# tokkiwa/FlashGMM

Measured on AMD Instinct MI355X. Metric: encode+decode Mpixels/s (Kodak, K=4 N=192) + GMM-CDF HBM GB/s vs roofline, higher is better.
Workload: dtype f32; 1 GPU; kodak24; schedule=codec, images_per_gpu=24, K=4, approx_mode=polya, param_dtype=f32, coded_symbols_per_gpu=6223104, streams_per_gpu=48, one_device_rehearsal=False

## Files before the change

flashgmm_amd/csrc/fgmm_capi.cpp:

```cpp
#include <sched.h>

#include <string>

#include "fgmm_ctx.h"

using namespace fgmm;

namespace fgmm {

static thread_local char t_err[512] = "";
char *last_error_buffer(size_t *cap) {
  if (cap) *cap = sizeof t_err;
  return t_err;
}
int fail(int code, const char *fmt, ...) {
  va_list ap;
  va_start(ap, fmt);
  vsnprintf(t_err, sizeof t_err, fmt, ap);
  va_end(ap);
  return code;
}

}

// ... 87 lines not shown
  m.ms[5] = tr.ms();
  m.worker_busy_ms = busy;
  m.worker_wait_ms = wait;
  for (int k = 0; k < 3; ++k) m.head_ms[k] = head ? head[k] : 0.0;
}
int fgmm_ctx::prof_begin(int which, dev::Stream s) {
  if (!profiling) return FGMM_OK;
  DEV_TRY(dev::event_record(prof[which][0], s));
  return FGMM_OK;
}
int fgmm_ctx::prof_end(int which, dev::Stream s) {
  if (!profiling) return FGMM_OK;
  DEV_TRY(dev::event_record(prof[which][1], s));
  prof_valid[which] = true;
  return FGMM_OK;
}

namespace {
bool mode_ok(int mode) { return mode >= 0 && mode <= 2; }
struct StagedRows {
  const float *s = nullptr, *m = nullptr, *w = nullptr;
  int64_t stride_n = 0, stride_k = 0;
};
}

extern "C" {

int fgmm_abi_version(void) { return FGMM_ABI_VERSION; }
const char *fgmm_last_error(void) { return fgmm::last_error_buffer(nullptr); }

namespace {
struct OptName {
  const char *name;
  int64_t fgmm_ctx::Opts::*field;
  int64_t lo, hi;
  const char *env;
};
const OptName kOpts[] = {
    {"pieces", &fgmm_ctx::Opts::pieces, 0, kMaxPieces, "FGMM_PIECES"},
    {"dec_first", &fgmm_ctx::Opts::dec_first, 1, 1 << 20, "FGMM_DEC_FIRST"},
    {"tab_cap_e", &fgmm_ctx::Opts::tab_cap_e, 256, 32768, "FGMM_TAB_CAP_E"},
    {"stage_max_mb", &fgmm_ctx::Opts::stage_max_mb, 0, 1 << 30, "FGMM_STAGE_MAX_MB"},
    {"trace", &fgmm_ctx::Opts::trace, 0, 2, "FGMM_TRACE"},
    {"enc_vec", &fgmm_ctx::Opts::enc_vec, 0, 8, "FGMM_VEC"},
    {"enc_linear", &fgmm_ctx::Opts::enc_linear, 0, 1, nullptr},
    {"ef_rows", &fgmm_ctx::Opts::ef_rows, 0, 2, "FGMM_EF_ROWS"},
    {"ef_min", &fgmm_ctx::Opts::ef_min, kTabEfMin, 1 << 20, "FGMM_EF_MIN_ROWS"},
    {"enc_ways", &fgmm_ctx::Opts::enc_ways, 0, kMaxEncWays, "FGMM_ENC_WAYS"},
    {"ckpt_decode", &fgmm_ctx::Opts::ckpt_decode, 0, 2, "FGMM_CKPT_DECODE"},
    {"spin_lat", &fgmm_ctx::Opts::spin_lat, -1, 1ll << 40, "FGMM_SPIN_LAT"},
    {"gpu_decode", &fgmm_ctx::Opts::gpu_decode, 0, 2, "FGMM_GPU_DECODE"},
    {"enc_segs", &fgmm_ctx::Opts::enc_segs, 0, 2, "FGMM_ENC_SEGS"},
    {"scatter_rounds", &fgmm_ctx::Opts::scatter_rounds, 0, 1, nullptr},
};
}

namespace {
double cgroup_cpu_quota() {
  double best = -1.0;
  auto take = [&best](double q) {
    if (q > 0 && (best < 0 || q < best)) best = q;
  };
  auto read_line = [](const std::string &path, char *buf, size_t cap) {
    FILE *f = fopen(path.c_str(), "r");
    if (!f) return false;
    const bool ok = fgets(buf, (int)cap, f) != nullptr;
    fclose(f);
    return ok;
  };
  char buf[256];
  std::string v2_rel, v1_rel;
  const std::string sysroot = getenv("FGMM_SYSROOT") ? getenv("FGMM_SYSROOT") : "";
  if (FILE *f = fopen((sysroot + "/proc/self/cgroup").c_str(), "r")) {
    while (fgets(buf, sizeof buf, f)) {
      std::string ln(buf);
      while (!ln.empty() && (ln.back() == '\n' || ln.back() == '\r')) ln.pop_back();
      const size_t a = ln.find(':'), b = a == std::string::npos ? a : ln.find(':', a + 1);
      if (b == std::string::npos) continue;
      const std::string ctrl = ln.substr(a + 1, b - a - 1), rel = ln.substr(b + 1);
      if (ctrl.empty()) v2_rel = rel;
      else if (("," + ctrl + ",").find(",cpu,") != std::string::npos) v1_rel = rel;
    }
    fclose(f);
  }
  for (const char *root : {"/sys/fs/cgroup", "/sys/fs/cgroup/unified"}) {
    std::string rel = v2_rel;
    for (;;) {
      if (read_line(sysroot + root + rel + (rel.empty() || rel.back() != '/' ? "/" : "") + "cpu.max", buf, sizeof buf)) {
        long long q = 0, p = 0;
        if (sscanf(buf, "%lld %lld", &q, &p) == 2 && q > 0 && p > 0) take((double)q / (double)p);
      }
      if (rel.empty() || rel == "/") break;
      const size_t cut = rel.find_last_of('/');
      rel = cut == std::string::npos ? std::string() : rel.substr(0, cut);
    }
  }
  for (const char *root : {"/sys/fs/cgroup/cpu", "/sys/fs/cgroup/cpu,cpuacct"}) {
    std::string rel = v1_rel;
    for (;;) {
      const std::string dir = sysroot + root + rel + (rel.empty() || rel.back() != '/' ? "/" : "");
      long long q = 0, p = 0;
      if (read_line(dir + "cpu.cfs_quota_us", buf, sizeof buf) && sscanf(buf, "%lld", &q) == 1 && q > 0 &&
          read_line(dir + "cpu.cfs_period_us", buf, sizeof buf) && sscanf(buf, "%lld", &p) == 1 && p > 0)
        take((double)q / (double)p);
      if (rel.empty() || rel == "/") break;
      const size_t cut = rel.find_last_of('/');
// ... 835 lines not shown
```

flashgmm_amd/csrc/fgmm_ctx.h:

```cpp
#pragma once
#include <math.h>
#include <pthread.h>
#include <sched.h>
#include <stdarg.h>
#include <stdio.h>
#include <stdlib.h>
#include <string.h>

#include <algorithm>
#include <atomic>
#include <chrono>
#include <condition_variable>
#include <functional>
#include <mutex>
#include <queue>
#include <string>
#include <thread>
#include <vector>

#include "../../include/flashgmm_amd.h"
#include "fgmm_device.h"
#include "fgmm_internal.h"

namespace fgmm {
// ... 240 lines not shown
CensusOff census_take(Arena &ar, int M);
void census_bind(EncDesc &d, const fgmm_ctx *ctx, const CensusOff &o);
void census_desc(EncDesc &d, const fgmm_ctx *ctx, const CensusOff &o, const float *y, const fgmm_params *params_or_null, int M, int64_t hw,
                 int clamp);
bool enc_vec4_ok(const EncDesc &d, const void *out, bool two_byte);
int census_side_info(const fgmm_ctx *ctx, const CensusOff &o, int M, int64_t hw, int64_t *zero_bitmap_or_null, int32_t *abs_max_out,
                     float *min_max_or_null = nullptr);

struct DeviceGuard {
  int prev = -1;
  bool ok = false;
  explicit DeviceGuard(int d) {
    if (dev::get_device(&prev) == 0 && (prev == d || dev::set_device(d) == 0)) ok = true;
  }
  ~DeviceGuard() {
    int cur;
    if (ok && prev >= 0 && dev::get_device(&cur) == 0 && cur != prev) (void)dev::set_device(prev);
  }
};

struct TempDevice {
  std::vector<void *> v;
  ~TempDevice() {
    for (void *p : v) (void)dev::free_device(p);
  }
  int alloc(size_t bytes, char **out) {
    void *p = nullptr;
    DEV_TRY(dev::malloc_device(&p, std::max<size_t>(bytes, 256)));
    v.push_back(p);
    *out = static_cast<char *>(p);
    return FGMM_OK;
  }
};

}

struct fgmm_ctx {
  int device = 0;
  std::mutex mu;
  fgmm::Pool *pool = nullptr;
  fgmm::WorkerCpus worker_cpus;
  fgmm::Pool *dec_pool = nullptr;
  fgmm::Pool *decoders() const { return dec_pool ? dec_pool : pool; }
  char *d_ws = nullptr;
  size_t d_cap = 0;
  char *h_ws = nullptr;
  size_t h_cap = 0;
  std::vector<fgmm::dev::Event> events;
  std::vector<fgmm::dev::Event> sleep_events;
  fgmm::dev::Stream copy_stream = nullptr;
  fgmm::dev::Stream aux_stream = nullptr;
  struct Opts {
    int64_t pieces = 0, dec_first = 2, tab_cap_e = fgmm::kTabCapE, stage_max_mb = 0, trace = 0, enc_vec = 0, enc_linear = 1, ef_rows = 0,
            ef_min = fgmm::kTabEfDefault, enc_ways = 0, ckpt_decode = 0, spin_lat = 400000, gpu_decode = 0, enc_segs = 1, scatter_rounds = 1;
  } opt;
  struct Chunk {
    char *p;
    size_t cap, used;
  };
  std::vector<Chunk> chunks;
  void chunks_reset() {
    for (auto &c : chunks) c.used = 0;
  }
  int chunk_alloc(size_t bytes, char **out);
  char *d_stage = nullptr;
  size_t d_stage_cap = 0;
  int ensure_stage(size_t bytes);
  void *d_xs = nullptr;
  size_t d_xs_cap = 0;
  uint32_t *d_rate_log2 = nullptr;
  size_t stage_budget() const;
  int ensure_streams();
  int ensure_device(size_t bytes);
  int ensure_host(size_t bytes);
  int ensure_events(size_t n, size_t n_sleep = 0);
  std::vector<int32_t> h_sym;
  void trim();
  const std::chrono::steady_clock::time_point born = std::chrono::steady_clock::now();
  static constexpr int kLogCap = 64;
  fgmm_call_marks log[kLogCap];
  unsigned long long log_n = 0;
  void log_call(int kind, int count, const fgmm::Trace &tr, const double ms[5], double busy, double wait, const double *head = nullptr);
  bool profiling = false;
  fgmm::dev::Event prof[4][2] = {{nullptr, nullptr}, {nullptr, nullptr}, {nullptr, nullptr}, {nullptr, nullptr}};
  bool prof_valid[4] = {false, false, false, false};
  int prof_begin(int which, fgmm::dev::Stream s);
  int prof_end(int which, fgmm::dev::Stream s);
  unsigned long long stat[6] = {0, 0, 0, 0, 0, 0};
};

namespace fgmm {

struct EncItem {
  bool latent = false;
  const float *y = nullptr;
  const float *x = nullptr;
  const void *xs = nullptr;
  const int32_t *sym_dev = nullptr;
  const int32_t *sym_host = nullptr;
  fgmm_params prm{};
  int64_t stride_p = 1;
  int32_t M = 0;
  int64_t hw = 0;
  int clamp = 0;
  float *yq = nullptr;
  fgmm_symbuf *symbuf = nullptr;
  int64_t ckpt_stride = 0;
// ... 164 lines not shown
```

flashgmm_amd/csrc/fgmm_decode_gpu.cpp:

```cpp
#include "fgmm_ctx.h"

namespace fgmm {

bool gpu_decodable(const DecItem &it, int64_t n) {
  return it.y_hat && !it.sym_host_out && it.ckpt && it.n_ckpt > 0 && it.ckpt_stride >= 256 && !(it.ckpt_stride & (it.ckpt_stride - 1)) &&
         n > 0 && it.n_ckpt == (n - 1) / it.ckpt_stride && it.n_ckpt < (1 << 24) && it.max_bs >= 0 && 2 * (int64_t)it.max_bs + 2 <= 2048  &&
         it.enc_len >= 8 && !(it.enc_len & 3) && it.stride_p == 1;
}

int decode_batch_gpu(fgmm_ctx *ctx, dev::Stream stream, std::vector<DecItem> &items, const std::vector<int> &which, int mode,
                     std::vector<int> &redo) {
  Trace tr("decode-gpu", (int)ctx->opt.trace);
  const int count = (int)which.size();
  const bool clamped = items[which[0]].clamp != 0, f16 = items[which[0]].prm.dtype == FGMM_F16;
  Arena ar;
  int64_t n_segs = 0;
  for (int k = 0; k < count; ++k) n_segs += items[which[k]].n_ckpt + 1;
  const size_t o_descs = ar.take(sizeof(SegDesc) * (size_t)count);
  const size_t o_segs = ar.take(sizeof(SegRef) * (size_t)n_segs);
  struct Off {
    size_t list, ckpt, words, status;
  };
  std::vector<Off> off((size_t)count);
  for (int k = 0; k < count; ++k) {
    DecItem &it = items[which[k]];
    off[(size_t)k].list = ar.take(sizeof(int32_t) * (size_t)std::max(it.M, 1), 16);
    off[(size_t)k].ckpt = ar.take(sizeof(fgmm_ckpt) * (size_t)it.n_ckpt, 16);
    off[(size_t)k].words = ar.take(it.enc_len, 16);
  }
  const size_t upload_bytes = ar.off;
  const size_t o_status = ar.take(sizeof(uint32_t) * (size_t)n_segs, 256);
  {
    size_t at = o_status;
    for (int k = 0; k < count; ++k) {
      off[(size_t)k].status = at;
      at += sizeof(uint32_t) * (size_t)(items[which[k]].n_ckpt + 1);
    }
  }
  int rc;
  if ((rc = ctx->ensure_device(ar.off)) || (rc = ctx->ensure_host(ar.off))) return rc;
  SegDesc *hd = reinterpret_cast<SegDesc *>(ctx->h_ws + o_descs);
  SegRef *hs = reinterpret_cast<SegRef *>(ctx->h_ws + o_segs);
  int64_t max_dead = 0;
  for (int k = 0; k < count; ++k) {
    DecItem &it = items[which[k]];
    int32_t *list = reinterpret_cast<int32_t *>(ctx->h_ws + off[(size_t)k].list);
    int r = 0, dead = it.n_ch;
    for (int c = 0; c < it.M; ++c) {
      if (!it.zero_bitmap || it.zero_bitmap[c] != 0) list[r++] = c;
      else list[dead++] = c;
    }
    max_dead = std::max<int64_t>(max_dead, it.M - it.n_ch);
    memcpy(ctx->h_ws + off[(size_t)k].ckpt, it.ckpt, sizeof(fgmm_ckpt) * (size_t)it.n_ckpt);
    memcpy(ctx->h_ws + off[(size_t)k].words, it.enc, it.enc_len);
    SegDesc &d = hd[k];
    memset(&d, 0, sizeof d);
    d.scales = it.prm.scales;
    d.means = it.prm.means;
    d.weights = it.prm.weights;
    d.stride_k = it.prm.stride_k;
    d.stride_c = it.prm.stride_c;
    d.stride_p = it.stride_p;
    d.hw = it.hw;
    d.n = it.n;
    d.chan_list = reinterpret_cast<const int32_t *>(ctx->d_ws + off[(size_t)k].list);
    d.max_bs = it.max_bs;
    d.clamp = it.clamp;
    d.logits = (it.prm.flags & FGMM_PARAMS_LOGITS) ? 1 : 0;
    d.words = reinterpret_cast<const uint32_t *>(ctx->d_ws + off[(size_t)k].words);
    d.n_words = (int64_t)(it.enc_len / 4);
    d.ckpt = reinterpret_cast<const fgmm_ckpt *>(ctx->d_ws + off[(size_t)k].ckpt);
    d.n_ckpt = it.n_ckpt;
    d.stride = it.ckpt_stride;
    d.y_hat = it.y_hat;
    d.status = reinterpret_cast<uint32_t *>(ctx->d_ws + off[(size_t)k].status);
    d.dead_list = d.chan_list + it.n_ch;
    d.n_dead = it.M - it.n_ch;
  }
  {
    constexpr int kBuckets = 256;
    std::vector<uint32_t> wgt((size_t)n_segs);
    uint32_t w_max = 1;
    int64_t at = 0;
    for (int k = 0; k < count; ++k) {
      const DecItem &it = items[which[k]];
      const uint64_t end_all = it.enc_len / 4 - 2;
      uint64_t prev = 0;
      for (int64_t sgm = 0; sgm <= it.n_ckpt; ++sgm) {
        const uint64_t pos = sgm < it.n_ckpt ? it.ckpt[sgm].pos : end_all;
        const uint64_t wds = pos >= prev ? pos - prev : 0;
        wgt[(size_t)at] = (uint32_t)std::min<uint64_t>(wds, 0x7FFFFFFFu);
        w_max = std::max(w_max, wgt[(size_t)at]);
        prev = pos;
        ++at;
      }
    }
    int64_t first[kBuckets + 1] = {};
    auto bucket = [&](uint32_t wv) { return kBuckets - 1 - (int)((uint64_t)wv * (kBuckets - 1) / w_max); };
    for (int64_t q = 0; q < n_segs; ++q) ++first[bucket(wgt[(size_t)q]) + 1];
    for (int b = 0; b < kBuckets; ++b) first[b + 1] += first[b];
    at = 0;
    for (int k = 0; k < count; ++k)
      for (int64_t sgm = 0; sgm <= items[which[k]].n_ckpt; ++sgm, ++at) hs[first[bucket(wgt[(size_t)at])]++] = SegRef{k, (int32_t)sgm};
  }
  DEV_TRY(dev::copy_async(ctx->d_ws, ctx->h_ws, upload_bytes, dev::kH2D, stream));
  LAUNCH_TRY(launch_segzero(reinterpret_cast<const SegDesc *>(ctx->d_ws + o_descs), count, max_dead, stream));
  if ((rc = ctx->prof_begin(3, stream))) return rc;
  LAUNCH_TRY(launch_segdec(reinterpret_cast<const SegDesc *>(ctx->d_ws + o_descs), reinterpret_cast<const SegRef *>(ctx->d_ws + o_segs), n_segs, mode_with_planes(mode, items[which[0]].prm.dtype),
                           clamped, f16, stream));
  if ((rc = ctx->prof_end(3, stream))) return rc;
  DEV_TRY(dev::copy_async(ctx->h_ws + o_status, ctx->d_ws + o_status, sizeof(uint32_t) * (size_t)n_segs, dev::kD2H, stream));
  tr.mark("enqueued");
  const double t_enq = tr.ms();
  DEV_TRY(dev::stream_sync(stream));
  tr.mark("segments decoded");
  {
    const double t_done = tr.ms(), mk[5] = {t_enq, t_enq, t_enq, t_done, t_done};
    ctx->log_call(2, count, tr, mk, 0.0, 0.0);
  }
  for (int k = 0; k < count; ++k) {
    DecItem &it = items[which[k]];
    const uint32_t *st = reinterpret_cast<const uint32_t *>(ctx->h_ws + off[(size_t)k].status);
    uint32_t worst = 0;
    for (int64_t sgm = 0; sgm <= it.n_ckpt; ++sgm) worst = std::max(worst, st[sgm]);
    if (worst != kSegOk) redo.push_back(which[k]);
    else it.status = FGMM_OK, it.done.store(1);
    if (tr.on && worst != kSegOk) {
      int64_t first = 0, n_bad = 0;
      for (int64_t sgm = it.n_ckpt; sgm >= 0; --sgm)
        if (st[sgm] != kSegOk) first = sgm, ++n_bad;
      fprintf(stderr, "[fgmm decode-gpu]   item %d: %lld of %lld segments not ok, the first: segment %lld status %u\n", which[k], (long long)n_bad,
              (long long)it.n_ckpt + 1, (long long)first, st[first]);
    }
  }
  ctx->stat[1] = 0;
  ctx->stat[2] = ctx->stat[3] = 0;
  ctx->stat[4] = (unsigned long long)(count - (int)redo.size());
  ctx->stat[5] = (unsigned long long)redo.size();
  for (int k = 0; k < count; ++k) ctx->stat[2] += (unsigned long long)items[which[k]].n;
  return FGMM_OK;
}

}
```

flashgmm_amd/csrc/fgmm_internal.h:

```cpp
#pragma once
#include <stddef.h>
#include <stdint.h>

#include "../../include/flashgmm_amd.h"

#if defined(__HIPCC__)
#define FGMM_HD __host__ __device__
#else
#define FGMM_HD
#endif

namespace fgmm {


struct EncDesc {
  const float *y;
  const int32_t *sym;
  const void *scales, *means, *weights;
  int64_t stride_k, stride_c, stride_p;
  int64_t hw;
  int32_t M;
  int32_t clamp;
  int32_t logits;
  uint32_t meta_slots;
// ... 93 lines not shown
  const float *anchors;
  float *out;
  const float *wp, *bp;
  int32_t M, c_out, h, w2, odd;
  int32_t mt, n_kt;
  int32_t pt;
};
int launch_ckbd_ctx_pack(const float *w, const float *bias_or_null, int M, int c_out, bool transposed, float *wp, float *bp, uint32_t *bad, void *stream);
int ckbd_ctx_tiles(int64_t n, int64_t pt, int c_out);
int launch_ckbd_ctx(const CkbdCtxArgs &args, int64_t n, void *stream);

constexpr int kCkbdWgradSliceMin = 256;
constexpr int kCkbdWgradSliceMax = 16;
struct CkbdWgradSlices { int64_t S, L; };
static inline CkbdWgradSlices ckbd_wgrad_slices(int64_t P) {
  if (P <= 0) return {0, 32};
  const int64_t want = (P + kCkbdWgradSliceMin - 1) / kCkbdWgradSliceMin, s0 = want < kCkbdWgradSliceMax ? want : kCkbdWgradSliceMax;
  const int64_t L = 32 * ((P + 32 * s0 - 1) / (32 * s0));
  return {(P + L - 1) / L, L};
}
static inline int64_t ckbd_wgrad_cols(int M) { return (int64_t)kCkbdCtxTaps * M + 1; }
struct CkbdWgradArgs {
  const float *anchors, *g;
  float *partial;
  int32_t M, c_out, h, w2, odd;
  int32_t mt;
  int32_t col0, n_col;
  int32_t P, L, S;
};
int ckbd_wgrad_tiles(int64_t S, int n_col, int c_out);
int launch_ckbd_wgrad(const CkbdWgradArgs &args, void *stream);
int launch_ckbd_wgrad_finish(const float *partial, int M, int c_out, int S, float *dweight_or_null, float *dbias_or_null, void *stream);

struct SegDesc {
  const void *scales, *means, *weights;
  int64_t stride_k, stride_c, stride_p;
  int64_t hw;
  int64_t n;
  const int32_t *chan_list;
  int32_t max_bs, clamp, logits, pad_;
  const uint32_t *words;
  int64_t n_words;
  const fgmm_ckpt *ckpt;
  int64_t n_ckpt, stride;
  float *y_hat;
  uint32_t *status;
  const int32_t *dead_list;
  int64_t n_dead;
};
struct SegRef {
  int32_t item, seg;
};
enum : uint32_t { kSegOk = 0, kSegMismatch = 1, kSegHard = 2, kSegStream = 3 };
int launch_segdec(const SegDesc *d_descs, const SegRef *d_segs, int64_t n_segs, int mode, bool clamped, bool f16, void *stream);
int launch_segzero(const SegDesc *d_descs, int count, int64_t max_dead, void *stream);

constexpr int kMaxPieces = 32;
constexpr int kAutoPiecesMax = 24;
constexpr int kEncSegs = 4;
constexpr int kTabEdgeSlots = 64;
constexpr int kTabCounters = 4 + kTabEdgeSlots;
#ifndef FGMM_EF_MIN
#define FGMM_EF_MIN 14
#endif
constexpr uint32_t kTabEfMin = FGMM_EF_MIN;
constexpr uint32_t kTabEfDefault = 33;
constexpr uint32_t kHdr2Escape = 255;
FGMM_HD static inline int32_t cvtt_i32(float f) {
  return (f > -2147483904.0f && f < 2147483648.0f) ? (int32_t)f : INT32_MIN;
}
FGMM_HD static inline uint32_t tab_hdr_pack(int32_t a, uint32_t cnt, uint32_t nonmono) {
  return (uint32_t)(uint16_t)(int16_t)a | ((cnt & 0x7FFFu) << 16) | (nonmono << 31);
}
FGMM_HD static inline int32_t tab_hdr_a(uint32_t h) { return (int32_t)(int16_t)(uint16_t)(h & 0xFFFFu); }
FGMM_HD static inline uint32_t tab_hdr_cnt(uint32_t h) { return (h >> 16) & 0x7FFFu; }
FGMM_HD static inline uint32_t tab_hdr_nonmono(uint32_t h) { return h >> 31; }
FGMM_HD static inline unsigned long long tab_hdr8_pack(int32_t a, uint32_t cnt, uint32_t nonmono) {
  return (unsigned long long)(uint32_t)a | ((unsigned long long)((cnt & 0x7FFFFFFFu) | (nonmono << 31)) << 32);
}
FGMM_HD static inline int32_t tab_hdr8_a(unsigned long long h) { return (int32_t)(uint32_t)h; }
FGMM_HD static inline uint32_t tab_hdr8_cnt(unsigned long long h) { return (uint32_t)(h >> 32) & 0x7FFFFFFFu; }
FGMM_HD static inline uint32_t tab_hdr8_nonmono(unsigned long long h) { return (uint32_t)(h >> 63); }
constexpr uint32_t kTabNoEf = 0x7FFFFFFFu;
FGMM_HD static inline bool tab_row_is_ef(uint32_t cnt, uint32_t nonmono, uint32_t ef_min) { return cnt >= ef_min && !nonmono; }
constexpr uint32_t kTabEf12Max = 48;
FGMM_HD static inline uint32_t tab_ef_l(uint32_t cnt) { return cnt <= kTabEf12Max ? 12u : 8u; }
FGMM_HD static inline uint32_t tab_ef_hb(uint32_t cnt, uint32_t l) { return cnt + (65536u >> l); }
FGMM_HD static inline uint32_t tab_ef_lb(uint32_t cnt, uint32_t l) { return (tab_ef_hb(cnt, l) + 7u) & ~7u; }
FGMM_HD static inline unsigned long long tab_ef_bits(uint32_t cnt, uint32_t l) { return (unsigned long long)cnt * l + tab_ef_lb(cnt, l); }
FGMM_HD static inline unsigned long long tab_row_bytes(uint32_t cnt, uint32_t nonmono, uint32_t ef_min) {
  return tab_row_is_ef(cnt, nonmono, ef_min) ? 2ull * ((tab_ef_bits(cnt, tab_ef_l(cnt)) + 15ull) >> 4) : 2ull * (unsigned long long)cnt;
}
FGMM_HD static inline bool tab_hdr_fits16(int32_t max_bs) { return 2 * (int64_t)max_bs + 2 <= 254; }
FGMM_HD static inline int tab_hdr_form(int32_t max_bs) { return tab_hdr_fits16(max_bs) ? 2 : (max_bs <= 16382 ? 4 : 8); }
constexpr int kTabCapE = 12288;
constexpr int kTabCapEWide = 16384;
constexpr int kTabMaxTl = 256;
FGMM_HD static inline int tab_tl(int32_t max_bs, int cap_e) {
  const int64_t W = 2 * (int64_t)max_bs + 2;
  const int64_t t = (cap_e / W) & ~15ll;
  return t >= 16 ? (int)(t > kTabMaxTl ? kTabMaxTl : t) : 0;
}

constexpr int kModeMask = 0xFF, kPlanesBf16 = 0x100;
static inline bool planes_two_byte(int dtype) { return dtype == FGMM_F16 || dtype == FGMM_BF16; }
static inline int mode_with_planes(int mode, int dtype) { return dtype == FGMM_BF16 ? (mode | kPlanesBf16) : mode; }
static inline int planes_of(int mode, bool f16) { return (mode & kPlanesBf16) ? FGMM_BF16 : (f16 ? FGMM_F16 : FGMM_F32); }
// ... 185 lines not shown
```

flashgmm_amd/csrc/fgmm_tab.hip:

```cpp
#include <algorithm>

#include "fgmm_decframe.h"

namespace fgmm {

template <int MODE, bool CLAMPED, typename PT> struct TabLatent {
  float mu[4], sg[4], pi[4], rs[4];
  int max_bs;

  __device__ __forceinline__ void load(const DecDesc &d, int c, int64_t p) {
    const int64_t base = (int64_t)c * d.stride_c + p * d.stride_p;
#pragma unroll
    for (int k = 0; k < 4; ++k) {
      const float s = ld1<PT>(d.scales, base + k * d.stride_k);
      sg[k] = CLAMPED ? clamp_scale(s) : s;
      rs[k] = CLAMPED ? rcp_refined(sg[k]) : 0.0f;
      mu[k] = ld1<PT>(d.means, base + k * d.stride_k);
      pi[k] = ld1<PT>(d.weights, base + k * d.stride_k);
    }
    if (d.logits) softmax4(pi);
    max_bs = d.max_bs;
  }
  __device__ __forceinline__ uint32_t edge(int j) const {
    const float x = (float)(j - max_bs) - 0.5f;
// ... 456 lines not shown
    auto unit = [&](uint32_t h) -> uint32_t {
      const bool escaped = d.hdr_form == 2 && R.nm;
      if (escaped && h < 2) return (tab_hdr_pack(R.a_idx - max_bs, R.cnt, 1u) >> (16 * h)) & 0xFFFFu;
      if (!R.efl) return R.entry(escaped ? h - 2 : h);
      const uint32_t bit0 = 16 * h;
      uint32_t v = 0;
      if (bit0 < R.HB) v = (S.bitmap[(R.aux >> 16) + (h >> 1)] >> (16 * (h & 1u))) & 0xFFFFu;
      if (bit0 + 16 > R.LB) {
        const int rel = (int)bit0 - (int)R.LB;
        uint32_t j = rel > 0 ? ((uint32_t)rel * R.M) >> 20 : 0u;
        const uint32_t mask = (1u << R.efl) - 1u;
        for (; j < R.cnt; ++j) {
          const int sh = (int)(j * R.efl) - rel;
          if (sh >= 16) break;
          const uint32_t lowbits = R.entry(j) & mask;
          v |= sh >= 0 ? lowbits << sh : lowbits >> -sh;
        }
        v &= 0xFFFFu;
      }
      return v;
    };
    for (; q < q_end; ++q) {
      uint32_t val = 0;
      if (4 * q < B) {
        if (4 * q >= r_end) {
          do {
            ++l;
            r_beg = r_end;
            r_end = S.rowoff[l + 1];
          } while (4 * q >= r_end);
          R.load(S, E16, l, d.ef_min);
        }
        const uint32_t h = (4 * q - r_beg) >> 1;
        val = unit(h);
        if (4 * q + 2 < r_end) {
          val |= unit(h + 1) << 16;
        } else if (4 * q + 2 < B) {
          ++l;
          r_beg = r_end;
          r_end = S.rowoff[l + 1];
          R.load(S, E16, l, d.ef_min);
          val |= unit(0) << 16;
        }
      }
      stg<uint32_t>(out + 4 * (size_t)q, val);
    }
  }
  TAB_T(5);
}

#ifdef FGMM_SEG_PROF
__device__ unsigned long long g_segprof[8];
__device__ unsigned long long g_segtimes[2 * 16384];
#define SEG_T(v) const unsigned long long v = clock64()
#define SEG_ACC(i, v) seg_acc[i] += (unsigned long long)(v)
#else
#define SEG_T(v)
#define SEG_ACC(i, v)
#endif
constexpr int kSegCapE = 2048;
constexpr int kSegBufE = 0;
constexpr int kSegBufPa = 2 * kSegCapE;
constexpr int kSegBufPb = kSegBufPa + 256;
constexpr int kSegBufPc = kSegBufPb + 256;
constexpr int kSegBufOut = kSegBufPc + 256;
constexpr int kSegBufNk = kSegBufOut + 512;
constexpr int kSegBufBytes = kSegBufNk + 16;
constexpr int kSegLdsP = 0;
constexpr int kSegLdsOff = 64 * 64;
constexpr int kSegLdsCtrl = kSegLdsOff + 4 * 68 + 3 * 4 * 64;
constexpr int kSegLdsBuf = kSegLdsCtrl + 32;
constexpr int kSegLds = kSegLdsBuf + 2 * kSegBufBytes;
#ifdef FGMM_SEG_WAVES
#define FGMM_SEG_OCC __attribute__((amdgpu_waves_per_eu(FGMM_SEG_WAVES, FGMM_SEG_WAVES)))
#else
#define FGMM_SEG_OCC
#endif
template <int MODE, bool CLAMPED, typename PT>
__global__ __launch_bounds__(192) FGMM_SEG_OCC void segdec_kernel(const SegDesc *__restrict__ descs, const SegRef *__restrict__ segs, int64_t n_segs) {
  __shared__ __attribute__((aligned(16))) unsigned char lds[kSegLds];
  float4_t *const P = reinterpret_cast<float4_t *>(lds + kSegLdsP);
  uint32_t *const offP = reinterpret_cast<uint32_t *>(lds + kSegLdsOff);
  uint32_t *const winL = offP + 68, *const tsfL = winL + 64;
  uint32_t *const nmL = tsfL + 64;
  volatile uint32_t *const ctrl = reinterpret_cast<volatile uint32_t *>(lds + kSegLdsCtrl);
  const int64_t wid = blockIdx.x;
  if (wid >= n_segs) return;
  const uint32_t lane = threadIdx.x & 63u;
  const int role = __builtin_amdgcn_readfirstlane((int)(threadIdx.x >> 6));
  const bool producer = role != 0;
  const bool two_producers = blockDim.x > 128;
  const SegRef ref = segs[wid];
  const SegDesc &d = descs[ref.item];
  const int64_t sg = ref.seg;
  const int64_t lo = sg * d.stride, hi = sg == d.n_ckpt ? d.n : lo + d.stride;
  const int32_t max_bs = d.max_bs;
  const int W = 2 * max_bs + 2;
  auto uni = [](uint32_t v) { return (uint32_t)__builtin_amdgcn_readfirstlane((int)v); };
  auto bcast = [](uint32_t v, uint32_t k) { return (uint32_t)__builtin_amdgcn_readlane((int)v, (int)k); };
  auto buf = [&](int n) { return lds + kSegLdsBuf + (n & 1) * kSegBufBytes; };
#ifdef FGMM_SEG_PROF
  unsigned long long seg_acc[6] = {};
#endif
  SEG_T(t_begin);
#ifdef FGMM_SEG_PROF
  const unsigned long long w_begin = wall_clock64();
#endif

  auto publish = [&](int slot, uint32_t v) {
    __builtin_amdgcn_fence(__ATOMIC_RELEASE, "workgroup");
    if (lane == 0) ctrl[slot] = v;
  };
  auto await = [&](int slot, uint32_t v) {
    for (int spins = 0; uni(ctrl[slot]) != v; ++spins) {
      __builtin_amdgcn_s_sleep(2);
      if (spins > (1 << 20)) {
        if (lane == 0) ctrl[6] = 1;
        break;
      }
    }
    __builtin_amdgcn_fence(__ATOMIC_ACQUIRE, "workgroup");
  };
  auto eval_pairs = [&](uint32_t t0, uint32_t t_end, int nk, uint32_t NP, uint32_t *E32) {
    int l = 0;
    uint32_t l_beg = 0, l_end = 0;
    uint32_t t = t0 + lane;
    if (t < t_end) {
      l = find_owner(offP, nk, t);
      l_beg = offP[l];
      l_end = l + 1 < nk ? offP[l + 1] : NP;
    }
    uint32_t carry = 0;
    for (; t < t_end; t += 64) {
      while (t >= l_end) {
        ++l;
        l_beg = l_end;
        l_end = l + 1 < nk ? offP[l + 1] : NP;
      }
      uint32_t wl, tl_, q0, q1;
      FGMM_DEC_EVAL_PAIR(MODE, CLAMPED, P, l, (wl = winL[l], tl_ = tsfL[l], (int)(wl & 0xFFFFu) + 2 * (int)(t - l_beg)), (tl_ >> 16) != 0, max_bs, q0, q1);
      const uint32_t pk = q0 | (q1 << 16);
      E32[t] = pk;
      const uint32_t before = (uint32_t)__builtin_amdgcn_update_dpp((int)carry, (int)pk, 0x138, 0xF, 0xF, false);
      const uint32_t prev = t > l_beg ? before >> 16 : 0u;
      if (prev > q0 || q0 > q1) nmL[l] = 1;
      carry = bcast(pk, 63u);
    }
  };
  auto seam = [](uint32_t NP) { return std::min(NP, ((NP * 7u) / 16u + 63u) & ~63u); };
  auto produce1 = [&](unsigned char *B, uint32_t seq) {
    await(2, seq);
    const int nk = (int)uni(ctrl[4]);
    const uint32_t NP = uni(ctrl[5]);
    eval_pairs(seam(NP), NP, nk, NP, reinterpret_cast<uint32_t *>(B + kSegBufE));
    __builtin_amdgcn_s_waitcnt(0xc07f);
    publish(3, seq);
  };
  auto produce = [&](int64_t base, unsigned char *B, uint32_t seq) {
    SEG_T(t_a);
    uint32_t *const E32 = reinterpret_cast<uint32_t *>(B + kSegBufE);
    const uint16_t *const E16 = reinterpret_cast<const uint16_t *>(E32);
    const int64_t i = std::min(base + lane, hi - 1);
    const int64_t cj = i / d.hw, p = i - cj * d.hw;
    const int c = dec_channel<true>(d, cj);
    float mu[4], sgm[4], pi[4], rs[4];
    bool tame;
    FGMM_DEC_PARAMS(CLAMPED, PT, d, c, p, mu, sgm, pi, rs, tame);
    int j_lo, j_hi;
    uint32_t T_sat;
    tab_window<MODE>(mu, sgm, pi, 1, max_bs, W, j_lo, j_hi, T_sat);
    FGMM_DEC_PARAMS_STORE(P, lane, mu, sgm, pi, rs);
    const uint32_t win = (uint32_t)j_lo | ((uint32_t)(j_hi - j_lo) << 16);
    const int nk_max = (int)std::min<int64_t>(64, hi - base);
    const uint32_t pairs = (int)lane < nk_max ? (uint32_t)(j_hi - j_lo + 1) >> 1 : 0u;
    uint32_t incl = pairs;
#pragma unroll
    for (int o = 1; o < 64; o <<= 1) {
      const uint32_t t = (uint32_t)__shfl_up((int)incl, o, 64);
      if (lane >= (uint32_t)o) incl += t;
    }
    const int nk = std::max(1, (int)__popcll(__ballot((int)lane < nk_max && 2 * incl <= (uint32_t)kSegCapE)));
    const uint32_t excl = incl - pairs;
    offP[lane] = excl;
    winL[lane] = win;
    tsfL[lane] = T_sat | (tame ? 0x10000u : 0u);
    nmL[lane] = 0;
    const uint32_t NP = bcast(incl, (uint32_t)(nk - 1));
    if (lane == 0) {
      offP[64] = NP;
      ctrl[4] = (uint32_t)nk;
      ctrl[5] = NP;
    }
    __builtin_amdgcn_s_waitcnt(0xc07f);
    __builtin_amdgcn_wave_barrier();
    if (two_producers) publish(2, seq);
    SEG_T(t_b);
    const uint32_t H = two_producers ? seam(NP) : NP;
    eval_pairs(0u, H, nk, NP, E32);
    __builtin_amdgcn_s_waitcnt(0xc07f);
    if (two_producers) await(3, seq);
    if (lane == 0 && H < NP) {
      const int l = find_owner(offP, nk, H);
      if (H > offP[l] && (E32[H - 1] >> 16) > (E32[H] & 0xFFFFu)) nmL[l] = 1;
    }
    __builtin_amdgcn_s_waitcnt(0xc07f);
    __builtin_amdgcn_wave_barrier();
    const uint32_t len_l = win >> 16, jl_l = win & 0xFFFFu;
    const bool tail_l = (int)(jl_l + len_l) < W;
    const bool mine = (int)lane < nk && len_l != 0;
    const uint32_t first_l = mine ? (uint32_t)E16[2u * excl] : 1u, last_l = mine ? (uint32_t)E16[2u * excl + len_l - 1u] : 0u;
    const uint32_t nm_l = nmL[lane];
    const bool slow_l = nm_l != 0 || len_l > 63u || (tail_l && T_sat < last_l) || (jl_l == 0 && first_l != 0);
    uint32_t *const Bw = reinterpret_cast<uint32_t *>(B);
    Bw[kSegBufPa / 4 + lane] = (2u * excl) | ((len_l & 0x7Fu) << 12) | ((uint32_t)((int)jl_l - 1 - max_bs) << 19);
    Bw[kSegBufPb / 4 + lane] = (tail_l ? T_sat : 0u) | (slow_l ? 0x10000u : 0u) | (nm_l ? 0x20000u : 0u) | (tail_l ? 0x40000u : 0u);
    Bw[kSegBufPc / 4 + lane] = win;
    reinterpret_cast<int64_t *>(B + kSegBufOut)[lane] = (int64_t)c * d.hw + p;
    if (lane == 0) Bw[kSegBufNk / 4] = (uint32_t)nk;
    SEG_T(t_e);
    SEG_ACC(0, t_b - t_a);
    SEG_ACC(1, t_e - t_b);
  };

  const uint32_t *__restrict__ w = d.words + 2;
  const int64_t nw = d.n_words - 2;
  uint32_t x_lo = 0, x_hi = 0, err = kSegOk, wv = 0, wp = 0, wleft = 0;
  int64_t wbase = 0;
  auto uni64 = [&](uint64_t v) { return ((uint64_t)uni((uint32_t)(v >> 32)) << 32) | uni((uint32_t)v); };
  if (!producer) {
    if (sg == 0) {
      x_lo = uni(ldg<uint32_t>(d.words));
      x_hi = uni(ldg<uint32_t>(d.words + 1));
    } else {
      const uint64_t cx = ldg<uint64_t>(&d.ckpt[sg - 1].x), cp = ldg<uint64_t>(&d.ckpt[sg - 1].pos);
      x_lo = uni((uint32_t)cx);
      x_hi = uni((uint32_t)(cx >> 32));
      wbase = (int64_t)uni64(cp);
    }
    if (wbase < 0 || wbase > nw) {
      err = kSegMismatch;
      wbase = 0;
    }
    wv = wbase + lane < nw ? ldg<uint32_t>(w + wbase + lane) : 0u;
    wleft = (uint32_t)std::min<int64_t>(nw - wbase, 0x7FFFFFFF);
  }
  uint32_t sout = 0;
  auto next_word = [&]() -> uint32_t {
    if (wp == 64) {
      wbase += 64;
      wv = wbase + lane < nw ? ldg<uint32_t>(w + wbase + lane) : 0u;
      wp = 0;
    }
    if (wleft == 0) sout = 1; else --wleft;
    const uint32_t r = bcast(wv, wp);
// ... 81 lines not shown
        uint32_t below = 0, last = 0, start = 0, next = 0;
        bool found = false, bad = (b & 0x20000u) != 0;
        for (int off = 0; off < len; off += 64) {
          const int q = off + (int)lane;
          const bool valid = q < len;
          const uint32_t Eq = valid ? (uint32_t)E16[e0 + (uint32_t)q] : 0x10000u;
          const uint32_t n_valid = (uint32_t)std::min(64, len - off);
          if (!found) {
            const uint32_t n_le = (uint32_t)__popcll(__ballot(valid && Eq <= cf));
            if (n_le < n_valid) {
              next = bcast(Eq, n_le);
              start = n_le ? bcast(Eq, n_le - 1) : last;
              found = true;
            }
            below += n_le;
          }
          last = bcast(Eq, n_valid - 1);
          if (found) {
            if (off + 64 < len) last = (uint32_t)E16[e0 + (uint32_t)len - 1u];
            break;
          }
        }
        bad = bad || (tail && tsat < last);
        if (!found) {
          start = last;
          next = tsat;
          bad = bad || !(tail && tsat > cf);
        }
        const int J = jl + (int)below - 1;
        const uint32_t freq = next - start;
        if (__builtin_expect(bad || J < 0 || J > W - 2 || freq == 0 || freq > 0xFFFFu, 0)) {
          bad_acc = 1;
          break;
        }
        value = J - max_bs;
        advance(freq, cf - start);
        x_lo = uni(x_lo);
        x_hi = uni(x_hi);
      }
      if (lane == (uint32_t)k) myval = value;
    }
    if (sout) err = kSegStream;
    else if (bad_acc) err = kSegHard;
    if (!err && (int)lane < nk) stg<float>(d.y_hat + reinterpret_cast<const int64_t *>(B + kSegBufOut)[lane], (float)myval);
    SEG_T(t_e);
    SEG_ACC(3, t_e - t_c);
    SEG_ACC(4, nk);
    SEG_ACC(5, 1);
  };

  if (threadIdx.x < 8) ctrl[threadIdx.x] = 0;
  __syncthreads();
  if (role == 1) produce(lo, buf(0), 1u);
  else if (role == 2) produce1(buf(0), 1u);
  else if (lane == 0) ctrl[0] = err;
  __syncthreads();
  int64_t base = lo;
  for (int n = 0;; ++n) {
    unsigned char *const B = buf(n);
    if (ctrl[n & 1]) break;
    const int nk = (int)uni(reinterpret_cast<const uint32_t *>(B)[kSegBufNk / 4]);
    const int64_t next = base + nk;
    if (producer) {
      if (next < hi) {
        if (role == 1) produce(next, buf(n + 1), (uint32_t)n + 2u);
        else produce1(buf(n + 1), (uint32_t)n + 2u);
      }
    } else {
      consume(B, nk);
      if (lane == 0) ctrl[(n + 1) & 1] = err;
    }
    SEG_T(t_w);
    __syncthreads();
    SEG_ACC(2, clock64() - t_w);
    if (next >= hi) break;
    base = next;
  }
  if (!producer) {
    if (!err && ctrl[6]) err = kSegHard;
    if (!err && sg < d.n_ckpt) {
      const uint64_t cx = ldg<uint64_t>(&d.ckpt[sg].x), cp = ldg<uint64_t>(&d.ckpt[sg].pos);
      const uint64_t x = ((uint64_t)x_hi << 32) | x_lo;
      if (x != cx || (uint64_t)(wbase + wp) != cp) err = kSegMismatch;
    }
    if (lane == 0) stg<uint32_t>(d.status + sg, err);
  }
#ifdef FGMM_SEG_PROF
  if (lane == 0) {
    for (int q = 0; q < 6; ++q) atomicAdd(&g_segprof[q], seg_acc[q]);
    if (!producer) {
      atomicAdd(&g_segprof[6], (unsigned long long)(clock64() - t_begin));
      atomicAdd(&g_segprof[7], 1ull);
      if (wid < 16384) g_segtimes[2 * wid] = w_begin, g_segtimes[2 * wid + 1] = wall_clock64();
    }
  }
#endif
}
#ifdef FGMM_SEG_PROF
extern "C" int fgmm_debug_segprof(unsigned long long *out, int reset) {
  int rc = (int)hipMemcpyFromSymbol(out, HIP_SYMBOL(g_segprof), sizeof(g_segprof));
  if (reset) {
    unsigned long long z[8] = {};
    rc |= (int)hipMemcpyToSymbol(HIP_SYMBOL(g_segprof), z, sizeof(z));
  }
  return rc;
}
extern "C" int fgmm_debug_segtimes(unsigned long long *out) { return (int)hipMemcpyFromSymbol(out, HIP_SYMBOL(g_segtimes), sizeof(g_segtimes)); }
#endif

static inline int launch_err() { return (int)hipGetLastError(); }

__global__ __launch_bounds__(kBlock) void segzero_kernel(const SegDesc *__restrict__ descs) {
  const SegDesc &d = descs[blockIdx.y];
  if ((int64_t)blockIdx.x >= d.n_dead) return;
  float *out = d.y_hat + (int64_t)ldg<int32_t>(d.dead_list + blockIdx.x) * d.hw;
  for (int64_t i = threadIdx.x; i < d.hw; i += kBlock) stg<float>(out + i, 0.0f);
}
int launch_segzero(const SegDesc *d_descs, int count, int64_t max_dead, void *stream) {
  if (count <= 0 || max_dead <= 0) return 0;
  if (max_dead > 0x7FFFFFFFll) return (int)hipErrorInvalidValue;
  for (int c0 = 0; c0 < count; c0 += 65535) {
    hipLaunchKernelGGL(segzero_kernel, dim3((unsigned)max_dead, (unsigned)std::min(count - c0, 65535)), dim3(kBlock), 0,
                       static_cast<hipStream_t>(stream), d_descs + c0);
    if (const int e = launch_err()) return e;
  }
  return 0;
}
int launch_segdec(const SegDesc *d_descs, const SegRef *d_segs, int64_t n_segs, int mode, bool clamped, bool f16, void *stream) {
  if (n_segs <= 0) return 0;
  if (n_segs > 0x7FFFFFFFll) return (int)hipErrorInvalidValue;
  const dim3 grid((unsigned)n_segs), block(n_segs <= 4096 ? 192 : 128);
  return dec_launch([&](auto r) {
    using R = decltype(r);
    hipLaunchKernelGGL((segdec_kernel<R::MODE, R::CLAMPED, typename R::PT>), grid, block, 0, (hipStream_t)stream, d_descs, d_segs, n_segs);
  }, mode, clamped, f16);
}

static int launch_cdftab_pass(const DecDesc *d_descs, int count, int n_ch_max, int64_t hw_max, int mode, bool clamped, bool f16,
                              int pass, void *stream) {
  if (count <= 0 || n_ch_max <= 0 || hw_max <= 0) return 0;
  hipStream_t s = (hipStream_t)stream;
  const dim3 grid((unsigned)((hw_max + kBlock - 1) / kBlock), (unsigned)n_ch_max, (unsigned)count);
  return dec_launch([&](auto r) {
    using R = decltype(r);
    if (pass & 1) {
      hipLaunchKernelGGL((cdftab_count_kernel<R::MODE, R::CLAMPED, typename R::PT>), grid, dim3(kBlock), 0, s, d_descs);
      hipLaunchKernelGGL(cdftab_scan_kernel, dim3((unsigned)count), dim3(kBlock), 0, s, d_descs);
    }
    if (pass & 2) hipLaunchKernelGGL((cdftab_fill_kernel<R::MODE, R::CLAMPED, typename R::PT>), grid, dim3(kBlock), 0, s, d_descs);
  }, mode, clamped, f16);
}
int launch_cdftab_count(const DecDesc *d_descs, int count, int n_ch_max, int64_t hw_max, int mode, bool clamped, bool f16,
                        void *stream) {
  return launch_cdftab_pass(d_descs, count, n_ch_max, hw_max, mode, clamped, f16, 1, stream);
}
int launch_cdftab_fill(const DecDesc *d_descs, int count, int n_ch_max, int64_t hw_max, int mode, bool clamped, bool f16,
                       void *stream) {
  return launch_cdftab_pass(d_descs, count, n_ch_max, hw_max, mode, clamped, f16, 2, stream);
}
int launch_cdftab(const DecDesc *d_descs, int count, int n_ch_max, int64_t hw_max, int mode, bool clamped, bool f16,
                  void *stream) {
  return launch_cdftab_pass(d_descs, count, n_ch_max, hw_max, mode, clamped, f16, 3, stream);
}

int launch_tab(const DecDesc *d_descs, int count, int blocks_max, int tl_max, int cap_e, int mode, bool clamped, bool f16,
               void *stream) {
  if (count <= 0 || blocks_max <= 0) return 0;
  if (tl_max < 1 || tl_max > kTabMaxTl || cap_e < 32 || cap_e > 32768 || (cap_e & 31) || tab_smem_bytes(tl_max, cap_e) > 160 * 1024) return (int)hipErrorInvalidValue;
  const dim3 grid((unsigned)blocks_max, (unsigned)count);
  const size_t lds = tab_smem_bytes(tl_max, cap_e);
  return dec_launch([&](auto r) {
    using R = decltype(r);
    hipLaunchKernelGGL((tab_kernel<R::MODE, R::CLAMPED, typename R::PT>), grid, dim3(kBlock), lds, (hipStream_t)stream, d_descs, tl_max, cap_e);
  }, mode, clamped, f16);
}

}
```

Measured before the change: 1062 Mpixels/s.

## Add three-producer segment decode variant and weight-class stream splitting

Adds a 256-thread variant of the segment decode kernel in which a third producer wave takes part of the pair evaluation, using a second seam point. By default it is used only when a batch has at most 1280 segments. An opt-in mode sorts segments into light, medium and heavy classes by words per checkpoint stride and launches each class with a different wave count on separate streams, joined with events. The goal is more intra-block parallelism for small batches and better balance of uneven segments, at the cost of a heavier kernel, more register and LDS pressure, and extra stream synchronisation.

Result: slower. 989.0 Mpixels/s (-6.9%).

```diff
diff --git a/flashgmm_amd/csrc/fgmm_capi.cpp b/flashgmm_amd/csrc/fgmm_capi.cpp
--- a/flashgmm_amd/csrc/fgmm_capi.cpp
+++ b/flashgmm_amd/csrc/fgmm_capi.cpp
@@ -163,6 +163,9 @@
     {"gpu_decode", &fgmm_ctx::Opts::gpu_decode, 0, 2, "FGMM_GPU_DECODE"},
     {"enc_segs", &fgmm_ctx::Opts::enc_segs, 0, 2, "FGMM_ENC_SEGS"},
     {"scatter_rounds", &fgmm_ctx::Opts::scatter_rounds, 0, 1, nullptr},
+    {"seg_shape", &fgmm_ctx::Opts::seg_shape, 0, 5, "FGMM_SEG_SHAPE"},
+    {"seg_light", &fgmm_ctx::Opts::seg_light, 0, 1 << 20, nullptr},
+    {"seg_heavy", &fgmm_ctx::Opts::seg_heavy, 0, 1 << 20, nullptr},
 };
 }
 
diff --git a/flashgmm_amd/csrc/fgmm_ctx.h b/flashgmm_amd/csrc/fgmm_ctx.h
--- a/flashgmm_amd/csrc/fgmm_ctx.h
+++ b/flashgmm_amd/csrc/fgmm_ctx.h
@@ -316,7 +316,8 @@
   fgmm::dev::Stream aux_stream = nullptr;
   struct Opts {
     int64_t pieces = 0, dec_first = 2, tab_cap_e = fgmm::kTabCapE, stage_max_mb = 0, trace = 0, enc_vec = 0, enc_linear = 1, ef_rows = 0,
-            ef_min = fgmm::kTabEfDefault, enc_ways = 0, ckpt_decode = 0, spin_lat = 400000, gpu_decode = 0, enc_segs = 1, scatter_rounds = 1;
+            ef_min = fgmm::kTabEfDefault, enc_ways = 0, ckpt_decode = 0, spin_lat = 400000, gpu_decode = 0, enc_segs = 1, scatter_rounds = 1,
+            seg_shape = 0, seg_light = fgmm::kSegLightBelow, seg_heavy = fgmm::kSegHeavyFrom;
   } opt;
   struct Chunk {
     char *p;
diff --git a/flashgmm_amd/csrc/fgmm_decode_gpu.cpp b/flashgmm_amd/csrc/fgmm_decode_gpu.cpp
--- a/flashgmm_amd/csrc/fgmm_decode_gpu.cpp
+++ b/flashgmm_amd/csrc/fgmm_decode_gpu.cpp
@@ -1,6 +1,22 @@
 #include "fgmm_ctx.h"
 
 namespace fgmm {
+
+void seg_classify(const uint32_t *wgt, const uint32_t *cls, int64_t n, int64_t light_below, int64_t heavy_from, int64_t *order, int64_t count[3]) {
+  constexpr int kBuckets = 256;
+  uint32_t w_max = 1;
+  for (int64_t q = 0; q < n; ++q) w_max = std::max(w_max, wgt[q]);
+  auto class_of = [&](int64_t q) { return (int64_t)cls[q] >= heavy_from ? 2 : ((int64_t)cls[q] < light_below ? 0 : 1); };
+  auto bucket = [&](int64_t q) { return (2 - class_of(q)) * kBuckets + kBuckets - 1 - (int)((uint64_t)wgt[q] * (kBuckets - 1) / w_max); };
+  std::vector<int64_t> first(3 * kBuckets + 1, 0);
+  count[0] = count[1] = count[2] = 0;
+  for (int64_t q = 0; q < n; ++q) {
+    ++first[(size_t)bucket(q) + 1];
+    ++count[class_of(q)];
+  }
+  for (int b = 0; b < 3 * kBuckets; ++b) first[(size_t)b + 1] += first[(size_t)b];
+  for (int64_t q = 0; q < n; ++q) order[first[(size_t)bucket(q)]++] = q;
+}
 
 bool gpu_decodable(const DecItem &it, int64_t n) {
   return it.y_hat && !it.sym_host_out && it.ckpt && it.n_ckpt > 0 && it.ckpt_stride >= 256 && !(it.ckpt_stride & (it.ckpt_stride - 1)) &&
@@ -77,10 +93,14 @@
     d.dead_list = d.chan_list + it.n_ch;
     d.n_dead = it.M - it.n_ch;
   }
-  {
-    constexpr int kBuckets = 256;
-    std::vector<uint32_t> wgt((size_t)n_segs);
-    uint32_t w_max = 1;
+  const bool shaped = launch_segdec_waves != nullptr;
+  const int shape = shaped ? (int)ctx->opt.seg_shape : 1;
+  const bool by_weight = shape == 5;
+  int64_t n_class[3] = {0, 0, 0};
+  {
+    std::vector<uint32_t> wgt((size_t)n_segs), cls((size_t)n_segs);
+    std::vector<SegRef> ref((size_t)n_segs);
+    std::vector<int64_t> order((size_t)n_segs);
     int64_t at = 0;
     for (int k = 0; k < count; ++k) {
       const DecItem &it = items[which[k]];
@@ -90,24 +110,59 @@
         const uint64_t pos = sgm < it.n_ckpt ? it.ckpt[sgm].pos : end_all;
         const uint64_t wds = pos >= prev ? pos - prev : 0;
         wgt[(size_t)at] = (uint32_t)std::min<uint64_t>(wds, 0x7FFFFFFFu);
-        w_max = std::max(w_max, wgt[(size_t)at]);
+        cls[(size_t)at] = (uint32_t)std::min<uint64_t>((uint64_t)wgt[(size_t)at] * 1024u / (uint64_t)it.ckpt_stride, 0x7FFFFFFFu);
+        ref[(size_t)at] = SegRef{k, (int32_t)sgm};
         prev = pos;
         ++at;
       }
     }
-    int64_t first[kBuckets + 1] = {};
-    auto bucket = [&](uint32_t wv) { return kBuckets - 1 - (int)((uint64_t)wv * (kBuckets - 1) / w_max); };
-    for (int64_t q = 0; q < n_segs; ++q) ++first[bucket(wgt[(size_t)q]) + 1];
-    for (int b = 0; b < kBuckets; ++b) first[b + 1] += first[b];
-    at = 0;
-    for (int k = 0; k < count; ++k)
-      for (int64_t sgm = 0; sgm <= items[which[k]].n_ckpt; ++sgm, ++at) hs[first[bucket(wgt[(size_t)at])]++] = SegRef{k, (int32_t)sgm};
+    seg_classify(wgt.data(), cls.data(), n_segs, by_weight ? ctx->opt.seg_light : 0, by_weight ? ctx->opt.seg_heavy : (int64_t)1 << 40, order.data(), n_class);
+    for (int64_t q = 0; q < n_segs; ++q) hs[q] = ref[(size_t)order[(size_t)q]];
   }
   DEV_TRY(dev::copy_async(ctx->d_ws, ctx->h_ws, upload_bytes, dev::kH2D, stream));
   LAUNCH_TRY(launch_segzero(reinterpret_cast<const SegDesc *>(ctx->d_ws + o_descs), count, max_dead, stream));
   if ((rc = ctx->prof_begin(3, stream))) return rc;
-  LAUNCH_TRY(launch_segdec(reinterpret_cast<const SegDesc *>(ctx->d_ws + o_descs), reinterpret_cast<const SegRef *>(ctx->d_ws + o_segs), n_segs, mode_with_planes(mode, items[which[0]].prm.dtype),
-                           clamped, f16, stream));
+  {
+    const SegDesc *d_descs = reinterpret_cast<const SegDesc *>(ctx->d_ws + o_descs);
+    const SegRef *d_segs = reinterpret_cast<const SegRef *>(ctx->d_ws + o_segs);
+    const int pmode = mode_with_planes(mode, items[which[0]].prm.dtype);
+    struct Part {
+      int64_t first, n;
+      int waves;
+    } part[3];
+    int n_part = 0;
+    if (by_weight) {
+      int64_t first = 0;
+      for (int c = 2; c >= 0; first += n_class[c], --c)
+        if (n_class[c]) part[n_part++] = Part{first, n_class[c], 2 + c};
+    } else {
+      part[n_part++] = Part{0, n_segs, shape == 0 ? (n_segs <= kSegFewMax ? 4 : 0) : (shape == 1 ? 0 : shape)};
+    }
+    dev::Stream side[2] = {nullptr, nullptr};
+    if (n_part > 1) {
+      if ((rc = ctx->ensure_streams()) || (rc = ctx->ensure_events(3))) return rc;
+      side[0] = ctx->copy_stream, side[1] = ctx->aux_stream;
+      DEV_TRY(dev::event_record(ctx->events[0], stream));
+    }
+    int forked = 0, err = 0;
+    for (int q = 0; q < n_part && !err; ++q) {
+      const bool last = q == n_part - 1;
+      const dev::Stream s = last ? stream : side[q];
+      if (!last) err = dev::stream_wait_event(s, ctx->events[0]);
+      if (!err)
+        err = shaped ? launch_segdec_waves(d_descs, d_segs + part[q].first, part[q].n, pmode, clamped, f16, part[q].waves, s)
+                     : launch_segdec(d_descs, d_segs, n_segs, pmode, clamped, f16, s);
+      if (!err && !last) {
+        forked = q + 1;
+        err = dev::event_record(ctx->events[1 + q], s);
+      }
+    }
+    for (int q = 0; q < forked && !err; ++q) err = dev::stream_wait_event(stream, ctx->events[1 + q]);
+    if (err) {
+      for (int q = 0; q < forked; ++q) (void)dev::stream_sync(side[q]);
+      DEV_TRY(err);
+    }
+  }
   if ((rc = ctx->prof_end(3, stream))) return rc;
   DEV_TRY(dev::copy_async(ctx->h_ws + o_status, ctx->d_ws + o_status, sizeof(uint32_t) * (size_t)n_segs, dev::kD2H, stream));
   tr.mark("enqueued");
@@ -142,3 +197,8 @@
 }
 
 }
+
+extern "C" __attribute__((visibility("default"))) void fgmm_debug_seg_classes(const uint32_t *wgt, int64_t n, int64_t light_below, int64_t heavy_from,
+                                                                               int64_t *order, int64_t *count3) {
+  fgmm::seg_classify(wgt, wgt, n, light_below, heavy_from, order, count3);
+}
diff --git a/flashgmm_amd/csrc/fgmm_internal.h b/flashgmm_amd/csrc/fgmm_internal.h
--- a/flashgmm_amd/csrc/fgmm_internal.h
+++ b/flashgmm_amd/csrc/fgmm_internal.h
@@ -169,7 +169,12 @@
   int32_t item, seg;
 };
 enum : uint32_t { kSegOk = 0, kSegMismatch = 1, kSegHard = 2, kSegStream = 3 };
+constexpr int64_t kSegFewMax = 1280;
+constexpr int64_t kSegLightBelow = 120, kSegHeavyFrom = 190;
+void seg_classify(const uint32_t *wgt, const uint32_t *cls, int64_t n, int64_t light_below, int64_t heavy_from, int64_t *order, int64_t count[3]);
 int launch_segdec(const SegDesc *d_descs, const SegRef *d_segs, int64_t n_segs, int mode, bool clamped, bool f16, void *stream);
+__attribute__((weak)) int launch_segdec_waves(const SegDesc *d_descs, const SegRef *d_segs, int64_t n_segs, int mode, bool clamped, bool f16, int waves,
+                                              void *stream);
 int launch_segzero(const SegDesc *d_descs, int count, int64_t max_dead, void *stream);
 
 constexpr int kMaxPieces = 32;
diff --git a/flashgmm_amd/csrc/fgmm_tab.hip b/flashgmm_amd/csrc/fgmm_tab.hip
--- a/flashgmm_amd/csrc/fgmm_tab.hip
+++ b/flashgmm_amd/csrc/fgmm_tab.hip
@@ -532,6 +532,7 @@
 #ifdef FGMM_SEG_PROF
 __device__ unsigned long long g_segprof[8];
 __device__ unsigned long long g_segtimes[2 * 16384];
+__device__ unsigned int g_segslot;
 #define SEG_T(v) const unsigned long long v = clock64()
 #define SEG_ACC(i, v) seg_acc[i] += (unsigned long long)(v)
 #else
@@ -556,8 +557,8 @@
 #else
 #define FGMM_SEG_OCC
 #endif
-template <int MODE, bool CLAMPED, typename PT>
-__global__ __launch_bounds__(192) FGMM_SEG_OCC void segdec_kernel(const SegDesc *__restrict__ descs, const SegRef *__restrict__ segs, int64_t n_segs) {
+template <int MODE, bool CLAMPED, typename PT, bool THREE>
+__global__ __launch_bounds__(THREE ? 256 : 192) FGMM_SEG_OCC void segdec_kernel(const SegDesc *__restrict__ descs, const SegRef *__restrict__ segs, int64_t n_segs) {
   __shared__ __attribute__((aligned(16))) unsigned char lds[kSegLds];
   float4_t *const P = reinterpret_cast<float4_t *>(lds + kSegLdsP);
   uint32_t *const offP = reinterpret_cast<uint32_t *>(lds + kSegLdsOff);
@@ -569,7 +570,7 @@
   const uint32_t lane = threadIdx.x & 63u;
   const int role = __builtin_amdgcn_readfirstlane((int)(threadIdx.x >> 6));
   const bool producer = role != 0;
-  const bool two_producers = blockDim.x > 128;
+  const bool two_producers = THREE || blockDim.x > 128;
   const SegRef ref = segs[wid];
   const SegDesc &d = descs[ref.item];
   const int64_t sg = ref.seg;
@@ -627,14 +628,17 @@
       carry = bcast(pk, 63u);
     }
   };
-  auto seam = [](uint32_t NP) { return std::min(NP, ((NP * 7u) / 16u + 63u) & ~63u); };
+  auto seam = [](uint32_t NP) { return std::min(NP, ((NP * (THREE ? 5u : 7u)) / 16u + 63u) & ~63u); };
+  auto seam2 = [](uint32_t NP, uint32_t s1) { return THREE ? std::min(NP, (s1 + ((NP - s1 + 1u) >> 1) + 63u) & ~63u) : NP; };
   auto produce1 = [&](unsigned char *B, uint32_t seq) {
     await(2, seq);
     const int nk = (int)uni(ctrl[4]);
     const uint32_t NP = uni(ctrl[5]);
-    eval_pairs(seam(NP), NP, nk, NP, reinterpret_cast<uint32_t *>(B + kSegBufE));
+    const uint32_t s1 = seam(NP), s2 = seam2(NP, s1);
+    const bool last = THREE && role == 3;
+    eval_pairs(last ? s2 : s1, last ? NP : s2, nk, NP, reinterpret_cast<uint32_t *>(B + kSegBufE));
     __builtin_amdgcn_s_waitcnt(0xc07f);
-    publish(3, seq);
+    publish(last ? 7 : 3, seq);
   };
   auto produce = [&](int64_t base, unsigned char *B, uint32_t seq) {
     SEG_T(t_a);
@@ -675,11 +679,13 @@
     __builtin_amdgcn_wave_barrier();
     if (two_producers) publish(2, seq);
     SEG_T(t_b);
-    const uint32_t H = two_producers ? seam(NP) : NP;
-    eval_pairs(0u, H, nk, NP, E32);
+    const uint32_t s1 = two_producers ? seam(NP) : NP;
+    eval_pairs(0u, s1, nk, NP, E32);
     __builtin_amdgcn_s_waitcnt(0xc07f);
     if (two_producers) await(3, seq);
-    if (lane == 0 && H < NP) {
+    if constexpr (THREE) await(7, seq);
+    const uint32_t H = THREE && lane != 0 ? seam2(NP, s1) : s1;
+    if (lane < (THREE ? 2u : 1u) && H < NP) {
       const int l = find_owner(offP, nk, H);
       if (H > offP[l] && (E32[H - 1] >> 16) > (E32[H] & 0xFFFFu)) nmL[l] = 1;
     }
@@ -867,7 +873,7 @@
   if (threadIdx.x < 8) ctrl[threadIdx.x] = 0;
   __syncthreads();
   if (role == 1) produce(lo, buf(0), 1u);
-  else if (role == 2) produce1(buf(0), 1u);
+  else if (role >= 2) produce1(buf(0), 1u);
   else if (lane == 0) ctrl[0] = err;
   __syncthreads();
   int64_t base = lo;
@@ -906,7 +912,8 @@
     if (!producer) {
       atomicAdd(&g_segprof[6], (unsigned long long)(clock64() - t_begin));
       atomicAdd(&g_segprof[7], 1ull);
-      if (wid < 16384) g_segtimes[2 * wid] = w_begin, g_segtimes[2 * wid + 1] = wall_clock64();
+      const unsigned int slot = atomicAdd(&g_segslot, 1u);
+      if (slot < 16384u) g_segtimes[2 * slot] = w_begin | ((unsigned long long)(blockDim.x >> 6) << 60), g_segtimes[2 * slot + 1] = wall_clock64();
     }
   }
 #endif
@@ -916,7 +923,9 @@
   int rc = (int)hipMemcpyFromSymbol(out, HIP_SYMBOL(g_segprof), sizeof(g_segprof));
   if (reset) {
     unsigned long long z[8] = {};
+    const unsigned int zero = 0;
     rc |= (int)hipMemcpyToSymbol(HIP_SYMBOL(g_segprof), z, sizeof(z));
+    rc |= (int)hipMemcpyToSymbol(HIP_SYMBOL(g_segslot), &zero, sizeof(zero));
   }
   return rc;
 }
@@ -942,12 +951,16 @@
   return 0;
 }
 int launch_segdec(const SegDesc *d_descs, const SegRef *d_segs, int64_t n_segs, int mode, bool clamped, bool f16, void *stream) {
+  return launch_segdec_waves(d_descs, d_segs, n_segs, mode, clamped, f16, 0, stream);
+}
+int launch_segdec_waves(const SegDesc *d_descs, const SegRef *d_segs, int64_t n_segs, int mode, bool clamped, bool f16, int waves, void *stream) {
   if (n_segs <= 0) return 0;
-  if (n_segs > 0x7FFFFFFFll) return (int)hipErrorInvalidValue;
-  const dim3 grid((unsigned)n_segs), block(n_segs <= 4096 ? 192 : 128);
+  if (n_segs > 0x7FFFFFFFll || (waves != 0 && (waves < 2 || waves > 4))) return (int)hipErrorInvalidValue;
+  const dim3 grid((unsigned)n_segs), block(waves ? 64u * (unsigned)waves : (n_segs <= 4096 ? 192u : 128u));
   return dec_launch([&](auto r) {
     using R = decltype(r);
-    hipLaunchKernelGGL((segdec_kernel<R::MODE, R::CLAMPED, typename R::PT>), grid, block, 0, (hipStream_t)stream, d_descs, d_segs, n_segs);
+    if (block.x == 256) hipLaunchKernelGGL((segdec_kernel<R::MODE, R::CLAMPED, typename R::PT, true>), grid, block, 0, (hipStream_t)stream, d_descs, d_segs, n_segs);
+    else hipLaunchKernelGGL((segdec_kernel<R::MODE, R::CLAMPED, typename R::PT, false>), grid, block, 0, (hipStream_t)stream, d_descs, d_segs, n_segs);
   }, mode, clamped, f16);
 }
 
```
